# MustaphaMensouri/Distributed-Continuous-Training-with-Airflow-PyTorch-Distributed-DDP-

Measured on AMD Instinct MI355X. Metric: samples/sec (whole node) for weather-MLP DDP, higher is better.
Workload: dtype fp32; 1 GPU; global_batch=4, per_rank_batch=4, parallelism=dp1, optimizer=adam lr=0.01, loss=ce, engine=fused-persistent, dataset_rows=8649, features=5

## Files before the change

distributed-continuous-training-with-airflow-pytorch-distributed-ddp-_amd/csrc/mlp_block5.hip:

```cpp
#include "knobs.h"
#include "mlp_block5_impl.h"
#include "mlp_select.h"

namespace dct {

void mlp_launch_block5_xg(int world, size_t bytes, hipStream_t st, const MlpShape& sh, const MlpArgs& a);
void mlp_launch_block5_b8(size_t bytes, hipStream_t st, const MlpShape& sh, const MlpArgs& a);

static bool b5_xg_world_ok(int w) { return w >= 2 && w <= 8; }

bool mlp_block5_two_micro(const MlpShape& sh, int B) { return B > blk5::B || sh.mlp_block == 8; }

bool mlp_block5_takes(const MlpShape& sh, const MlpLaunchKey& k) {
  const bool aligned = (sh.woff[1] % 4) == 0 && k.p_aligned && k.mv_aligned;
  const bool xg_ok = k.xg_world <= 1 ||
                     (k.mode == 0 && b5_xg_world_ok(k.xg_world) && k.xg_rank >= 0 && k.xg_rank < k.xg_world &&
                      k.xg_bufs && (!k.prof || k.xg_world == 2 || k.xg_world == 4 || k.xg_world == 8));
  const bool b8_ok = !mlp_block5_two_micro(sh, k.B) || !k.prof;
  return aligned && b8_ok && mlp_block5_shape_ok(sh.dims, sh.L, k.B) &&
         ((k.mode == 0 && !k.cursor) || (k.mode == 1 && k.steps == 1 && k.grad_out)) &&
         (k.loss_kind == 0 || k.loss_kind == 1) && !k.pending && (!k.stage || k.mode == 1) && xg_ok;
}

bool mlp_block5_xg_shape_ok(const MlpShape& sh, const MlpLaunchKey& k) {
  return k.mode == 0 && mlp_block5_shape_ok(sh.dims, sh.L, k.B) && mlp_block5_xg_bytes(k.xg_world) > 0;
}

bool mlp_block5_shape_ok(const int* dims, int L, int B) {
  return L == 3 && dims[1] == blk5::H && dims[2] == blk5::H && dims[0] >= 1 && dims[0] <= blk5::DMAX &&
         dims[3] == blk5::C && B >= 1 && B <= blk5::BMAX;
}

size_t mlp_block5_xg_bytes(int world) {
  switch (world) {
    case 2: return (size_t)b5x::Lay<2>::BYTES;
    case 4: return (size_t)b5x::Lay<4>::BYTES;
    case 8: return (size_t)b5x::Lay<8>::BYTES;
    case 3: return (size_t)b5x::Lay<3>::BYTES;
    case 5: return (size_t)b5x::Lay<5>::BYTES;
    case 6: return (size_t)b5x::Lay<6>::BYTES;
    case 7: return (size_t)b5x::Lay<7>::BYTES;
    default: return 0;
  }
}

template <bool WD, int LK, bool PROF = false>
static void b5_launch_sched(int sched, size_t bytes, hipStream_t st, const MlpShape& sh, const MlpArgs& a) {
  using namespace blk5;
  if (sched == 0) return b5_launch<WD, LK, PROF>(bytes, st, sh, a);
#ifdef B5_SCHED_AB
  if constexpr (!WD && LK == 0 && !PROF) {
    constexpr int D = SCHED_DEFAULT;
    constexpr int R = SCHED_R10, E = SCHED_R11;
    constexpr int masks[] = {R, R | SCH_PF_W0, R | SCH_ADAM_SM, R | SCH_DZ2F, R | SCH_DROP_INT, R | SCH_DB2,
                             E & ~SCH_PF_W0,
                             E, E | SCH_LOGIT_RS, E | SCH_INV_BS, E | SCH_ADAM_B02, D & ~SCH_INV_BS};
    bool done = false;
    b5x::static_for<sizeof(masks) / sizeof(masks[0])>([&](auto i) {
      constexpr int M = masks[decltype(i)::value];
      if (!done && sched == B5_SCHED_AB_BASE + M && M != D) {
        b5_launch<WD, LK, false, true, true, 1, -1, 1, M>(bytes, st, sh, a);
        done = true;
      }
    });
    if (done) return;
  }
#endif
  b5_launch<WD, LK, PROF, true, true, 1, -1, 1, SCHED_DEFAULT>(bytes, st, sh, a);
}

hipError_t mlp_launch_block5(const MlpShape& sh, const MlpArgs& a, hipStream_t st) {
  const size_t bytes = (size_t)blk5::LDS_FLOATS * sizeof(float);
  const bool wd = a.wd != 0.f;
  const int sched = knobs().b5_sched;
  if (!mlp_block5_takes(sh, mlp_launch_key(a))) return hipErrorInvalidValue;
  if (mlp_block5_two_micro(sh, a.B)) {
    mlp_launch_block5_b8(bytes, st, sh, a);
  } else if (a.xg_world > 1) {
    mlp_launch_block5_xg(a.xg_world, bytes, st, sh, a);
  } else if (a.mode == 1) {
    if (a.loss_kind == 0) b5_launch<false, 0, false, true, false>(bytes, st, sh, a);
    else b5_launch<false, 1, false, true, false>(bytes, st, sh, a);
  } else if (a.prof) {
    if (a.loss_kind == 0) b5_launch_sched<true, 0, true>(sched, bytes, st, sh, a);
    else b5_launch_sched<true, 1, true>(sched, bytes, st, sh, a);
  } else if (a.loss_kind == 0) {
    if (wd) b5_launch_sched<true, 0>(sched, bytes, st, sh, a);
    else b5_launch_sched<false, 0>(sched, bytes, st, sh, a);
  } else {
    if (wd) b5_launch_sched<true, 1>(sched, bytes, st, sh, a);
    else b5_launch_sched<false, 1>(sched, bytes, st, sh, a);
  }
  return hipGetLastError();
}

}
```

distributed-continuous-training-with-airflow-pytorch-distributed-ddp-_amd/csrc/mlp_block5_impl.h:

```cpp
#pragma once
#include <type_traits>

#include "mlp_block_util.h"

namespace dct {

namespace blk5 {
constexpr int H = 128, NT = 512, NW = 8, KS = 16, DMAX = 8, B = 4, C = 2, MBMAX = 2, BMAX = B * MBMAX;
constexpr int PSTR = 36;
template <int MB>
struct Lds {
  static constexpr int RB = B * MB;
  static constexpr int XT = 0;
  static constexpr int LAB = XT + 3 * DMAX * RB;
  static constexpr int MSK = LAB + (MB == 1 ? 16 : 32);
  static constexpr int LOGP = MSK + 2 * NW * 2;
  static constexpr int H1W = LOGP + 2 * NW * 8;
  static constexpr int H1X = H1W + MB * NW * KS * 4;
  static constexpr int PART = H1X + NW * KS * 4;
  static constexpr int W2L = PART + 2 * H * PSTR;
  static constexpr int B2L = W2L + 2 * H * C;
  static constexpr int ABT = B2L + 8;
  static constexpr int TOTAL = ABT + 4;
  static constexpr int DZF = TOTAL;
  static constexpr int TOTAL_DZF = DZF + 2 * H * 4;
  static_assert((DZF % 4) == 0, "16-B aligned");
  static_assert((H1W % 4) == 0 && (PART % 4) == 0 && (MSK % 4) == 0 && (LAB % 4) == 0 && (W2L % 4) == 0 &&
                    (B2L % 4) == 0 && (H1X % 4) == 0 && (LOGP % 4) == 0,
                "16-B aligned tiles");
};
static_assert(Lds<1>::TOTAL == 11036, "the batch <= 4 layout is round 5's");
constexpr int STG = H * H;
constexpr int LDS_FLOATS = Lds<MBMAX>::TOTAL > 2 * STG ? Lds<MBMAX>::TOTAL : 2 * STG;
static_assert(Lds<1>::TOTAL_DZF <= LDS_FLOATS, "SCH_DZ2F's region inside the launch's LDS");
static_assert(LDS_FLOATS * 4 <= 160 * 1024, "fits the CU");
using Stg = bku::Stage<H, NT>;
constexpr float LOG2E = 1.4426950408889634f, LN2 = 0.6931471805599453f;
constexpr int SCH_DROP = 1, SCH_ADAM_TAB = 2, SCH_WT1 = 8, SCH_WT2 = 16, SCH_WTB = 32;
constexpr int SCH_PRIO_LAT = 64;
constexpr int SCH_PF_W0 = 128, SCH_ADAM_SM = 256, SCH_DZ2F = 512, SCH_DROP_INT = 1024, SCH_DB2 = 2048;
constexpr int SCHED_R10 = SCH_DROP | SCH_ADAM_TAB | SCH_WTB | SCH_PRIO_LAT;
constexpr int SCHED_R11 = SCHED_R10 | SCH_PF_W0 | SCH_ADAM_SM | SCH_DZ2F | SCH_DROP_INT | SCH_DB2;
constexpr int SCH_LOGIT_RS = 4096, SCH_INV_BS = 8192, SCH_ADAM_B02 = 16384;
constexpr int SCHED_DEFAULT = SCHED_R11 | SCH_LOGIT_RS | SCH_INV_BS | SCH_ADAM_B02;
static_assert(SCHED_DEFAULT < 32768, "item masks stay below B5_SCHED_AB_BASE (knobs.h)");
}

namespace b5x {
typedef unsigned int v4u __attribute__((ext_vector_type(4)));
constexpr int SYS = 17;
constexpr int NP = 16, NS = 2;
constexpr int G = blk5::NT * 16;
template <int XW>
struct Lay {
  static constexpr int NO = (NP + XW - 1) / XW;
  static constexpr int RSS = NO + NS;
  static constexpr int AG = 2 * XW * RSS * G;
  static constexpr int LS = AG + 2 * (NP + NS) * G;
  static constexpr int EP = LS + ((2 * XW * 16 + 255) & ~255);
  static constexpr int BYTES = EP + (NP + NS) * 2 * G;
  static __device__ __forceinline__ int rs(int par, int src, int slot) { return ((par * XW + src) * RSS + slot) * G; }
  static __device__ __forceinline__ int ag(int par, int slot) { return AG + (par * (NP + NS) + slot) * G; }
  static __device__ __forceinline__ int ls(int par, int src) { return LS + (par * XW + src) * 16; }
  static __device__ __forceinline__ int ep(int slot, int mv) { return EP + (slot * 2 + mv) * G; }
};
__device__ __forceinline__ void put(__amdgpu_buffer_rsrc_t rs, int off, float x, float y, uint32_t tag) {
  v4u d;
  d.x = __float_as_uint(x);
  d.y = tag;
  d.z = __float_as_uint(y);
  d.w = tag;
  __builtin_amdgcn_raw_buffer_store_b128(d, rs, off, 0, SYS);
}
__device__ __forceinline__ bool get(__amdgpu_buffer_rsrc_t rs, int off, uint32_t tag, float& x, float& y) {
  const v4u d = __builtin_amdgcn_raw_buffer_load_b128(rs, off, 0, SYS);
  x = __uint_as_float(d.x);
  y = __uint_as_float(d.z);
  return (d.y == tag) & (d.w == tag);
}
template <int XW, class T>
__device__ __forceinline__ T pick(const T* v, int rank) {
  T r = v[0];
#pragma unroll
  for (int k = 1; k < XW; ++k) r = rank == k ? v[k] : r;
  return r;
}
template <int V>
using IC = std::integral_constant<int, V>;
template <int N, int I = 0, class F>
__device__ __host__ __forceinline__ void static_for(F&& f) {
  if constexpr (I < N) {
    f(IC<I>{});
    static_for<N, I + 1>(f);
  }
}
}

#define B5STAMP(k)                                              \
  if constexpr (PROF) {                                         \
    const unsigned long long t_ = __builtin_amdgcn_s_memtime(); \
    pacc[(k)] += t_ - t_last;                                   \
    t_last = t_;                                                \
  }

#define B5PRIO(p)                      \
  if constexpr (S_PLAT) {              \
    __builtin_amdgcn_sched_barrier(0); \
    __builtin_amdgcn_s_setprio(p);     \
    __builtin_amdgcn_sched_barrier(0); \
  }

__device__ __forceinline__ uint32_t b5_elem(int li, int r, int u) {
  return ((uint32_t)((li * 64 + r) * 65536 + u) + 0x165667B1u) * 0xC2B2AE3Du;
}
__device__ __forceinline__ float b5_drop(uint32_t seed, uint32_t gstep, uint32_t elem, float p, float scale) {
  uint32_t h = (seed * 0x9E3779B1u) ^ ((gstep + 0x7F4A7C15u) * 0x85EBCA77u);
  h ^= elem;
  h ^= h >> 16;
  h *= 0x7feb352du;
  h ^= h >> 15;
  h *= 0x846ca68bu;
  h ^= h >> 16;
  return u01(h) < p ? 0.f : scale;
}
__device__ __forceinline__ uint32_t b5_drop_thr(float p) { return (uint32_t)ceilf(p * 16777216.0f); }
__device__ __forceinline__ float b5_drop_int(uint32_t seed, uint32_t gstep, uint32_t elem, uint32_t thr, float scale) {
  uint32_t h = (seed * 0x9E3779B1u) ^ ((gstep + 0x7F4A7C15u) * 0x85EBCA77u);
  h ^= elem;
  h ^= h >> 16;
  h *= 0x7feb352du;
  h ^= h >> 15;
  h *= 0x846ca68bu;
  h ^= h >> 16;
  return (h >> 8) < thr ? 0.f : scale;
}

template <bool WD>
__device__ __forceinline__ void adam_pair(float& p0, float g0, float& m0, float& v0, float& p1, float g1, float& m1,
                                          float& v1, float b1, float b2, float wd, float A, float E) {
  if constexpr (WD) { g0 = fmaf(wd, p0, g0); g1 = fmaf(wd, p1, g1); }
  m0 = fmaf(b1, m0, g0);
  m1 = fmaf(b1, m1, g1);
  v0 = fmaf(b2, v0, g0 * g0);
  v1 = fmaf(b2, v1, g1 * g1);
  const float d0 = fmaf(__builtin_amdgcn_sqrtf(v0), A, E), d1 = fmaf(__builtin_amdgcn_sqrtf(v1), A, E);
  const float R = __builtin_amdgcn_rcpf(d0 * d1);
  p0 = fmaf(-m0, d1 * R, p0);
  p1 = fmaf(-m1, d0 * R, p1);
}

__device__ __forceinline__ bku::f32x4_t quad_transpose_mf(const float (&v)[4], const float (&e)[4]) {
  bku::f32x4_t t = (bku::f32x4_t){0.f, 0.f, 0.f, 0.f};
#pragma unroll
  for (int i = 0; i < 4; ++i) t = bku::mfma4(v[i], e[i], t);
  return t;
}

__device__ __forceinline__ float rs_bits2to5(float (&P)[16], int lane) {
  using namespace bku;
#pragma unroll
  for (int i = 0; i < 8; ++i) P[i] = swap32_sum(P[i], P[i + 8]);
#pragma unroll
  for (int i = 0; i < 4; ++i) P[i] = swap16_sum(P[i], P[i + 4]);
  const bool b3 = (lane >> 3) & 1, b2 = (lane >> 2) & 1;
#pragma unroll
  for (int i = 0; i < 2; ++i) {
    const float keep = b3 ? P[i + 2] : P[i], send = b3 ? P[i] : P[i + 2];
    P[i] = keep + dpp<ROR8>(send);
  }
  const float keep = b2 ? P[1] : P[0], send = b2 ? P[0] : P[1];
  const float t4 = dpp<ROR4>(send), t12 = dpp<0x12C>(send);
  return keep + (b2 ? t4 : t12);
}

typedef float v2f __attribute__((ext_vector_type(2)));
template <bool WD>
__device__ __forceinline__ void adam_v2(v2f& p, v2f g, v2f& m, v2f& v, float b1, float b2, float wd, float A, float E) {
  if constexpr (WD) g = (v2f)(wd) * p + g;
  m = (v2f)(b1) * m + g;
  v = (v2f)(b2) * v + g * g;
  const v2f sq = (v2f){__builtin_amdgcn_sqrtf(v.x), __builtin_amdgcn_sqrtf(v.y)};
  const v2f d = sq * (v2f)(A) + (v2f)(E);
  const float R = __builtin_amdgcn_rcpf(d.x * d.y);
  p = p - m * ((v2f){d.y, d.x} * R);
}
template <bool WD>
__device__ __forceinline__ void adam_v2r(v2f& p, v2f g, v2f& m, v2f& v, float b1, float b2, float wd, float A, float E) {
  if constexpr (WD) g = (v2f)(wd) * p + g;
  m = (v2f)(b1) * m + g;
  v = (v2f)(b2) * v + g * g;
  const v2f sq = (v2f){__builtin_amdgcn_sqrtf(v.x), __builtin_amdgcn_sqrtf(v.y)};
  const v2f d = sq * (v2f)(A) + (v2f)(E);
  p = p - m * (v2f){__builtin_amdgcn_rcpf(d.x), __builtin_amdgcn_rcpf(d.y)};
}

template <bool WD, int LK, bool PROF = false, bool DXM = true, bool ADAM = true, int XW = 1, int RK = -1, int MB = 1,
          int SCH = 0>
__global__ __launch_bounds__(blk5::NT, 1) void mlp_block5_kernel(MlpShape sh, MlpArgs a) {
  using namespace blk5;
  using namespace bku;
  static_assert(XW == 1 || (ADAM && XW >= 2 && XW <= 8), "exchange: train mode, 2..8 ranks");
  static_assert(MB >= 1 && MB <= MBMAX, "micro-batches per step");
  static_assert(SCH == 0 || (XW == 1 && MB == 1 && ADAM), "step-schedule items: one-rank train mode, one micro-batch");
  constexpr bool S_DROP = (SCH & SCH_DROP) != 0, S_TAB = (SCH & SCH_ADAM_TAB) != 0;
  constexpr int HQ = DXM ? (SCH / SCH_WT1) & 3 : 0;
  constexpr int HB = DXM ? (SCH / SCH_WTB) & 1 : 0;
  static_assert(HQ + HB <= KS / 4, "W1 has four k-blocks per wave");
  constexpr bool S_PLAT = (SCH & SCH_PRIO_LAT) != 0;
  constexpr bool S_PF = (SCH & SCH_PF_W0) != 0, S_SM = (SCH & SCH_ADAM_SM) != 0, S_DZF = (SCH & SCH_DZ2F) != 0;
  constexpr bool S_DINT = (SCH & SCH_DROP_INT) != 0, S_DB2 = (SCH & SCH_DB2) != 0;
  constexpr bool S_LRS = (SCH & SCH_LOGIT_RS) != 0, S_INVB = (SCH & SCH_INV_BS) != 0, S_B02 = (SCH & SCH_ADAM_B02) != 0;
  constexpr bool S_EV = S_SM || S_B02;
  using LY = Lds<MB>;
  constexpr int RB = LY::RB, XT = LY::XT, LAB = LY::LAB, MSK = LY::MSK, LOGP = LY::LOGP, H1W = LY::H1W;
  constexpr int H1X = LY::H1X, PART = LY::PART, W2L = LY::W2L, B2L = LY::B2L, ABT = LY::ABT, TOTAL = LY::TOTAL;
  constexpr int PS = XW > 1 ? 32 : 16;
  using XL = b5x::Lay<XW>;
  constexpr int NO = XL::NO;
  extern __shared__ __attribute__((aligned(16))) float lds[];
  const int tid = threadIdx.x, w = tid >> 6, l = tid & 63;
  const int D0 = sh.dims[0];
  const int r0 = l & 3;
  const int u = KS * w + (l >> 2);
  const int wo0 = sh.woff[0], bo0 = sh.boff[0], wo1 = sh.woff[1], bo1 = sh.boff[1];
  const int wo2 = sh.woff[2], bo2 = sh.boff[2];
  unsigned long long pacc[PROF ? PS : 1] = {};
  unsigned long long t_last = PROF ? __builtin_amdgcn_s_memtime() : 0ull;
  const unsigned long long t_kstart = t_last;

  const int Bsz = a.B;
  const int fb = tid & (RB - 1), fd = tid / RB;
  const int nel = Bsz * D0;
  int role = 0, pb = 0, pk = 0;
  if (tid < nel) { role = 1; pb = tid / D0; pk = tid - pb * D0; }
  else if (tid < nel + Bsz) { role = 2; pb = tid - nel; }
  const bool stp = !ADAM && a.stage != nullptr;
  uint32_t st_tag = 0u, st_x = 0u, st_lab = 0u;
  if (stp) {
    st_tag = a.stage[0];
    if (tid < RB * DMAX && fd < D0 && fb < Bsz) st_x = a.stage[64 + fb * D0 + fd];
    if (tid < Bsz) st_lab = a.stage[64 + nel + tid];
  }
  const int cur0 = (!ADAM && a.cursor) ? sload(a.cursor) : 0;
  const int bs0 = min(Bsz, a.n_items - cur0 * Bsz);
  const bool first_ok = tid < RB * DMAX && fb < bs0;
  const int rb_raw = a.idx[max(0, min(cur0 * Bsz + (first_ok ? fb : 0), a.n_items - 1))];
  const int rb_first = (first_ok && !stp) ? rb_raw : 0;
  int ridx_next = 0;
  if (!stp && role && (cur0 + 1) * Bsz + pb < a.n_items) ridx_next = a.idx[(cur0 + 1) * Bsz + pb];

  v4f sp[Stg::LD], sm[Stg::LD], sv[Stg::LD];
#pragma unroll
  for (int i = 0; i < Stg::LD; ++i) {
    const int f = wo1 + 4 * (i * NT + tid);
    sp[i] = *reinterpret_cast<const v4f*>(a.p + f);
    if constexpr (ADAM) sm[i] = *reinterpret_cast<const v4f*>(a.m + f);
  }
  if constexpr (ADAM) {
#pragma unroll
    for (int i = 0; i < Stg::LD; ++i) sv[i] = *reinterpret_cast<const v4f*>(a.v + wo1 + 4 * (i * NT + tid));
  }
  float w0[2], m0[2], v0[2];
#pragma unroll
  for (int i = 0; i < 2; ++i) {
    const int d = r0 + 4 * i;
    const bool ok = d < D0;
    const int f = wo0 + u * D0 + (ok ? d : 0);
    w0[i] = ok ? a.p[f] : 0.f;
    m0[i] = (ok && ADAM) ? a.m[f] : 0.f;
    v0[i] = (ok && ADAM) ? a.v[f] : 0.f;
  }
  float pb0 = a.p[bo0 + u], mb0 = ADAM ? a.m[bo0 + u] : 0.f, vb0 = ADAM ? a.v[bo0 + u] : 0.f;
  float pw2[C];
#pragma unroll
  for (int c = 0; c < C; ++c) pw2[c] = a.p[wo2 + c * H + u];
  const bool own_w2 = r0 < C;
  const int fw2 = wo2 + (XW > 1 ? (r0 & 1) : (own_w2 ? r0 : 0)) * H + u;
  float mw2 = ((own_w2 || XW > 1) && ADAM) ? a.m[fw2] : 0.f, vw2 = ((own_w2 || XW > 1) && ADAM) ? a.v[fw2] : 0.f;
  float pb1 = a.p[bo1 + u], mb1 = ADAM ? a.m[bo1 + u] : 0.f, vb1 = ADAM ? a.v[bo1 + u] : 0.f;
  const bool own_b2 = w == 0 && l < C;
  const int fb2 = bo2 + (own_b2 ? l : 0);
  float pb2 = own_b2 ? a.p[fb2] : 0.f, mb2 = (own_b2 && ADAM) ? a.m[fb2] : 0.f, vb2 = (own_b2 && ADAM) ? a.v[fb2] : 0.f;
  const int fbx = r0 == 0 ? bo0 + u : (r0 == 1 ? bo1 + u : bo2 + (l & 1));
  float pbx = 0.f, mbx = 0.f, vbx = 0.f;
  if constexpr (XW > 1) {
    pbx = a.p[fbx];
    mbx = a.m[fbx];
    vbx = a.v[fbx];
  }

  int t0 = a.t0;
  uint32_t step_base = a.step_base;
  if (a.step_counter) {
    t0 = sload(a.step_counter);
    step_base = (uint32_t)t0;
// ... 59 lines not shown
  const float sqc2 = XW > 1 ? a.k_sqc2 : sqrtf(c2);
#pragma unroll
  for (int j = 0; j < 2; ++j)
#pragma unroll
    for (int k = 0; k < KS; ++k) { m1[j][k] *= rc1; v1[j][k] *= rc2; }
#pragma unroll
  for (int i = 0; i < 2; ++i) { m0[i] *= rc1; v0[i] *= rc2; }
  mb0 *= rc1; vb0 *= rc2; mw2 *= rc1; vw2 *= rc2; mb1 *= rc1; vb1 *= rc2; mb2 *= rc1; vb2 *= rc2;
  mbx *= rc1; vbx *= rc2;
  v2f W[2][KS / 2], Mo[2][KS / 2], Vo[2][KS / 2];
#pragma unroll
  for (int j = 0; j < 2; ++j)
#pragma unroll
    for (int h = 0; h < KS / 2; ++h) {
      W[j][h] = (v2f){w1[j][2 * h], w1[j][2 * h + 1]};
      Mo[j][h] = (v2f){m1[j][2 * h], m1[j][2 * h + 1]};
      Vo[j][h] = (v2f){v1[j][2 * h], v1[j][2 * h + 1]};
    }
  const v2f z2 = (v2f){0.f, 0.f};
  v2f PSm = S_SM ? (v2f){0.f, pb1} : z2, MSm = S_SM ? (v2f){mw2, mb1} : z2, VSm = S_SM ? (v2f){vw2, vb1} : z2;
  v2f PW0 = S_SM ? (v2f){w0[0], w0[1]} : z2, MW0 = S_SM ? (v2f){m0[0], m0[1]} : z2, VW0 = S_SM ? (v2f){v0[0], v0[1]} : z2;
  v2f PB02 = S_B02 ? (v2f){pb0, pb2} : z2, MB02 = S_B02 ? (v2f){mb0, mb2} : z2, VB02 = S_B02 ? (v2f){vb0, vb2} : z2;
  const uint32_t inv_bsz = S_INVB ? __builtin_amdgcn_readfirstlane(
                                        __float_as_uint(__builtin_amdgcn_rcpf((float)(Bsz > 0 ? Bsz : 1))))
                                  : 0u;
  const int xrank = XW > 1 ? (RK >= 0 ? RK : a.xg_rank) : 0;
  v2f MoO[NO], VoO[NO];
  __amdgpu_buffer_rsrc_t xrr = __builtin_amdgcn_make_buffer_rsrc((void*)a.xg_recv, 0, 0, 0x00020000), xpr[XW];
  const bool sown = XW == 1 || (__builtin_amdgcn_readfirstlane(w) % XW) == xrank;
  bool xbad = false;
  unsigned long long xticks = 0;
  if constexpr (XW > 1) {
#pragma unroll
    for (int t = 0; t < NO; ++t) {
      v2f cm[XW], cv[XW];
#pragma unroll
      for (int k = 0; k < XW; ++k) {
        const int i = XW * t + k < b5x::NP ? XW * t + k : 0;
        cm[k] = Mo[i >> 3][i & 7];
        cv[k] = Vo[i >> 3][i & 7];
      }
      MoO[t] = b5x::pick<XW>(cm, xrank);
      VoO[t] = b5x::pick<XW>(cv, xrank);
    }
  }
  if constexpr (XW > 1) {
    xrr = __builtin_amdgcn_make_buffer_rsrc((void*)a.xg_recv, 0, XL::BYTES, 0x00020000);
#pragma unroll
    for (int q = 0; q < XW; ++q)
      xpr[q] = __builtin_amdgcn_make_buffer_rsrc((void*)sload_ptr(a.xg_peers, q), 0, XL::BYTES, 0x00020000);
  }
  auto xwait = [&](uint32_t tag, auto&& sweep) -> bool {
    const unsigned long long t_start = __builtin_amdgcn_s_memrealtime();
    for (int spin = 0;; ++spin) {
      asm volatile("" ::: "memory");
      if (__all(sweep())) return true;
      if ((spin & 15) == 15 && (long long)(__builtin_amdgcn_s_memrealtime() - t_start) > a.xg_timeout) {
        if (l == 0) __hip_atomic_store(a.xg_status, tag, __ATOMIC_RELAXED, __HIP_MEMORY_SCOPE_SYSTEM);
        return false;
      }
      __builtin_amdgcn_s_sleep(1);
    }
  };
  const int tb = tid * 16;
  uint32_t el0[MB], el1[MB];
  float f1[MB], f2[MB];
#pragma unroll
  for (int hf = 0; hf < MB; ++hf) {
    el0[hf] = b5_elem(0, r0 + B * hf, u);
    el1[hf] = b5_elem(1, r0 + B * hf, u);
    f1[hf] = b5_drop(a.seed, step_base, el0[hf], p_drop, scale);
    f2[hf] = b5_drop(a.seed, step_base, el1[hf], p_drop, scale);
  }
  const bool pf_wave = !S_PF || __builtin_amdgcn_readfirstlane(w) == 0;
  float* h1x = lds + H1X + w * (KS * 4);
  float eye[4];
#pragma unroll
  for (int i = 0; i < 4; ++i) eye[i] = r0 == i ? 1.f : 0.f;
  const int cb = (l >> 2) & 1;
  int xb = 0;
  float tabA = 0.f, tabE = 0.f;
  if (a.tune == 1 && w >= NW / 2) __builtin_amdgcn_s_setprio(1);
  if (a.tune == 2 && w < NW / 2) __builtin_amdgcn_s_setprio(1);
  if constexpr (PROF) {
    t_last = __builtin_amdgcn_s_memtime();
    pacc[9] = t_last - t_kstart;
  }
  for (int s = 0; s < a.steps; ++s) {
    const int sb = s + cur0;
    const int bs = min(Bsz, a.n_items - sb * Bsz);
    const uint32_t gstep = step_base + (uint32_t)s;
    const int xbn = xb == 2 ? 0 : xb + 1;
    const int pbuf = s & 1, nbuf = pbuf ^ 1;
    const float* xT = lds + XT + xb * DMAX * RB;
    const bool have_next = (s + 1 < a.steps);
    const int bs_next = have_next ? min(Bsz, a.n_items - (sb + 1) * Bsz) : 0;
    uint32_t raw_next = 0u;
    int ridx_next2 = 0;
    if constexpr (S_PF) {
      if (pf_wave) {
        raw_next = pf_base[(size_t)(uint32_t)ridx_next * (uint32_t)pf_stride];
        const int nx2 = min((sb + 2) * Bsz + pb, a.n_items - 1);
        ridx_next2 = a.idx[nx2 < 0 ? 0 : nx2];
      }
    } else {
      raw_next = pf_base[(size_t)ridx_next * pf_stride];
      const int nx2 = min((sb + 2) * Bsz + pb, a.n_items - 1);
      ridx_next2 = a.idx[nx2 < 0 ? 0 : nx2];
    }
    const uint32_t xtag = gstep + 1u;
    const int xpar = (int)(gstep & 1u);
    const int t = t0 + s + 1;
    float dz2m[MB][2][4];
    float dz = 0.f, xbl = 0.f, tls = 0.f;
    float h2 = 0.f, h1 = 0.f;
    float gw0s = 0.f, gw1s = 0.f, gb1s = 0.f, gbs = 0.f, g0s = 0.f, g1s = 0.f, db0s = 0.f;
    float aA = 0.f, aE = 0.f, aEv = 0.f;
    float f1n = 0.f, f2n = 0.f;
    f32x4_t wth[HQ + HB > 0 ? HQ + HB : 1][2];
    v2f GO[NO];
#pragma unroll
    for (int t2 = 0; t2 < NO; ++t2) GO[t2] = (v2f){0.f, 0.f};
    float xg_own = 0.f, xg_bx = 0.f;
    v2f xs_g0 = (v2f){0.f, 0.f}, xs_g1 = (v2f){0.f, 0.f};
    bool abort_step = false;
    auto dw1_pass = [&]() {
#pragma unroll
      for (int q = 0; q < KS / 4; ++q) {
        f32x4_t g[2];
#pragma unroll
        for (int j = 0; j < 2; ++j) g[j] = (f32x4_t){0.f, 0.f, 0.f, 0.f};
#pragma unroll
        for (int hf = 0; hf < MB; ++hf) {
          const float4 hq = *reinterpret_cast<const float4*>(lds + H1W + (hf * NW + w) * (KS * 4) + (4 * q + r0) * 4);
          const float hv[4] = {hq.x, hq.y, hq.z, hq.w};
#pragma unroll
          for (int j = 0; j < 2; ++j)
#pragma unroll
            for (int r = 0; r < 4; ++r) g[j] = mfma4(hv[r], dz2m[hf][j][r], g[j]);
        }

        if constexpr (ADAM && XW > 1) {
#pragma unroll
          for (int j = 0; j < 2; ++j)
#pragma unroll
            for (int h = 0; h < 2; ++h) {
              const int i = 8 * j + 2 * q + h;
              const float gx = g[j][2 * h], gy = g[j][2 * h + 1];
              if ((i % XW) == xrank) GO[i / XW] = (v2f){gx, gy};
              else b5x::put(xpr[i % XW], XL::rs(xpar, (xrank - i % XW + XW) % XW, i / XW) + tb, gx, gy, xtag);
            }
        } else if constexpr (ADAM) {
#pragma unroll
          for (int j = 0; j < 2; ++j)
#pragma unroll
            for (int h = 0; h < 2; ++h)
              adam_v2<WD>(W[j][2 * q + h], (v2f){g[j][2 * h], g[j][2 * h + 1]}, Mo[j][2 * q + h], Vo[j][2 * q + h], a.b1,
                          a.b2, a.wd, aA, aE);
        } else {
#pragma unroll
          for (int j = 0; j < 2; ++j)
            *reinterpret_cast<float4*>(a.grad_out + wo1 + (l + 64 * j) * H + KS * w + 4 * q) =
                make_float4(g[j][0], g[j][1], g[j][2], g[j][3]);
        }
      }
    };

#pragma unroll
    for (int hf = 0; hf < MB; ++hf) {
      const bool last = hf == MB - 1;
      const int mpar = MB == 1 ? pbuf : hf;
      float* h1w = lds + H1W + (hf * NW + w) * (KS * 4);

      const float4 xa = *reinterpret_cast<const float4*>(xT + r0 * RB + B * hf);
      const float4 xc = *reinterpret_cast<const float4*>(xT + (r0 + 4) * RB + B * hf);
      {
        const float wa = S_SM ? PW0.x : w0[0], wc = S_SM ? PW0.y : w0[1];
        const float acc0 = wa * xa.x + wc * xc.x, acc1 = wa * xa.y + wc * xc.y;
        const float acc2 = wa * xa.z + wc * xc.z, acc3 = wa * xa.w + wc * xc.w;
        const bool qb1 = (r0 >> 1) & 1, qb0 = r0 & 1;
        const float k0 = qb1 ? acc2 : acc0, k1 = qb1 ? acc3 : acc1;
        const float s0 = qb1 ? acc0 : acc2, s1 = qb1 ? acc1 : acc3;
        const float e0 = k0 + dpp<QP_X2>(s0), e1 = k1 + dpp<QP_X2>(s1);
        const float kq = qb0 ? e1 : e0, sq = qb0 ? e0 : e1;
        h1 = fmaxf(kq + dpp<QP_X1>(sq) + (S_B02 ? PB02.x : pb0), 0.f) * f1[hf];
        h1w[l] = h1;
        h1x[r0 * KS + (l >> 2)] = h1;
      }
      __builtin_amdgcn_wave_barrier();
      B5STAMP(0)
      {
        f32x4_t cq[2][KS / 4];
#pragma unroll
        for (int q = 0; q < KS / 4; ++q) {
          const float4 hq = *reinterpret_cast<const float4*>(h1x + r0 * KS + 4 * q);
          const float hv[4] = {hq.x, hq.y, hq.z, hq.w};
#pragma unroll
          for (int j = 0; j < 2; ++j) {
            cq[j][q] = (f32x4_t){0.f, 0.f, 0.f, 0.f};
#pragma unroll
            for (int e = 0; e < 4; ++e) cq[j][q] = mfma4(hv[e], W[j][2 * q + (e >> 1)][e & 1], cq[j][q]);
          }
        }
        f32x4_t cj[2];
#pragma unroll
        for (int j = 0; j < 2; ++j) cj[j] = (cq[j][0] + cq[j][1]) + (cq[j][2] + cq[j][3]);
        float* part = lds + PART + mpar * (H * PSTR);
#pragma unroll
        for (int j = 0; j < 2; ++j)
          *reinterpret_cast<float4*>(part + (l + 64 * j) * PSTR + w * 4) = make_float4(cj[j][0], cj[j][1], cj[j][2], cj[j][3]);
      }
      if (hf == 0) {
        if (stp) {
          const int bs_st = min(Bsz, a.n_items - (sb + 1) * Bsz);
          if (role) a.stage[64 + tid] = pb < bs_st ? raw_next : 0u;
          if (tid == 0) a.stage[0] = bs_st > 0 ? (uint32_t)(sb + 2) : 0u;
        }
        if (pf_wave) {
          if (role) {
            const uint32_t v = (have_next && pb < bs_next) ? raw_next : 0u;
            uint32_t* dst = (role == 1) ? reinterpret_cast<uint32_t*>(lds + XT + xbn * DMAX * RB) + pk * RB + pb
                                        : reinterpret_cast<uint32_t*>(lds + LAB) + xbn * RB + pb;
            *dst = v;
          }
          ridx_next = role ? ridx_next2 : 0;
        }
      }
      B5STAMP(1)
      lds_barrier();
      B5STAMP(2)
      B5PRIO(1)
      if constexpr (XW > 1) {
        if (lds[ABT] != 0.f) {
          abort_step = true;
          break;
        }
      }

      const float2 wv0 = *reinterpret_cast<const float2*>(lds + W2L + pbuf * (H * C) + l * C);
      const float2 wv1 = *reinterpret_cast<const float2*>(lds + W2L + pbuf * (H * C) + (l + 64) * C);
      const float b2c = lds[B2L + pbuf * 4 + cb];
      const int lab = reinterpret_cast<const int*>(lds + LAB)[xb * RB + B * hf + r0];
      {
        const float* pr = lds + PART + mpar * (H * PSTR) + u * PSTR + r0;
        float q[NW];
#pragma unroll
        for (int ww = 0; ww < NW; ++ww) q[ww] = pr[4 * ww];
        if constexpr (SCH != 0) {
          __builtin_amdgcn_sched_barrier(0);
          if constexpr (HQ > 0) {
#pragma unroll
            for (int qq = 0; qq < HQ; ++qq)
#pragma unroll
              for (int j = 0; j < 2; ++j) {
                const float wq[4] = {W[j][2 * qq].x, W[j][2 * qq].y, W[j][2 * qq + 1].x, W[j][2 * qq + 1].y};
                wth[qq][j] = quad_transpose_mf(wq, eye);
              }
          }
          if constexpr (S_DROP) {
            uint32_t gnext = gstep + 1u;
            asm volatile("" : "+s"(gnext));
            if constexpr (S_DINT) {
              f1n = b5_drop_int(a.seed, gnext, el0[0], drop_thr, scale);
              f2n = b5_drop_int(a.seed, gnext, el1[0], drop_thr, scale);
            } else {
              f1n = b5_drop(a.seed, gnext, el0[0], p_drop, scale);
              f2n = b5_drop(a.seed, gnext, el1[0], p_drop, scale);
            }
            asm volatile("" : "+v"(f1n), "+v"(f2n));
          }
          if constexpr (S_TAB) {
            const int ti = s & 63;
// ... 231 lines not shown
#pragma unroll
          for (int j = 0; j < 2; ++j) {
            const float wq[4] = {W[j][2 * q].x, W[j][2 * q].y, W[j][2 * q + 1].x, W[j][2 * q + 1].y};
            const f32x4_t wt = q < HQ + HB ? wth[q < HQ + HB ? q : 0][j] : quad_transpose_mf(wq, eye);
            acc[j] = (f32x4_t){0.f, 0.f, 0.f, 0.f};
#pragma unroll
            for (int i = 0; i < 4; ++i) acc[j] = mfma4(wt[i], dzt[j][i], acc[j]);
          }
          const f32x4_t at = acc[0] + acc[1];
#pragma unroll
          for (int m = 0; m < 4; ++m) P[4 * q + m] = at[m];
        }
        dz1 = rs_bits2to5(P, l);
      } else {
#pragma unroll
        for (int p = 0; p < 4; ++p) {
          float P[16];
#pragma unroll
          for (int kk = 0; kk < KS; ++kk)
            P[kk] = W[0][kk >> 1][kk & 1] * dz2m[hf][0][p] + W[1][kk >> 1][kk & 1] * dz2m[hf][1][p];
          const float tot = rs_small<16>(P, l);
          if (r0 == p) dz1 = tot;
        }
      }
      dz1 = h1 > 0.f ? dz1 * scale : 0.f;
      B5PRIO(1)
      {
        const float dq0 = dpp<QB0>(dz1), dq1 = dpp<QB1>(dz1), dq2 = dpp<QB2>(dz1), dq3 = dpp<QB3>(dz1);
        const float g0h = dq0 * xa.x + dq1 * xa.y + dq2 * xa.z + dq3 * xa.w;
        const float g1h = dq0 * xc.x + dq1 * xc.y + dq2 * xc.z + dq3 * xc.w;
        const float dbh = (dq0 + dq1) + (dq2 + dq3);
        g0s = hf == 0 ? g0h : g0s + g0h;
        g1s = hf == 0 ? g1h : g1s + g1h;
        db0s = hf == 0 ? dbh : db0s + dbh;
        if (last) {
          const float g0 = g0s, g1 = g1s;
          if constexpr (ADAM && XW > 1) {
            if (r0 == 0) xg_bx = db0s;
            xs_g0 = (v2f){g0, g1};
            xs_g1 = (v2f){xg_own, xg_bx};
            if (!sown) {
#pragma unroll
              for (int q = 0; q < XW; ++q)
                if (q == __builtin_amdgcn_readfirstlane(w) % XW) {
                  const int rel = (xrank - q + XW) % XW;
                  b5x::put(xpr[q], XL::rs(xpar, rel, NO) + tb, g0, g1, xtag);
                  b5x::put(xpr[q], XL::rs(xpar, rel, NO + 1) + tb, xg_own, xg_bx, xtag);
                }
            }
          } else if constexpr (ADAM) {
            if constexpr (S_SM)
              adam_v2<WD>(PW0, (v2f){g0, g1}, MW0, VW0, a.b1, a.b2, a.wd, aA, aEv);
            else
              adam_pair<WD>(w0[0], g0, m0[0], v0[0], w0[1], g1, m0[1], v0[1], a.b1, a.b2, a.wd, aA, aE);
            if constexpr (S_B02) {
              adam_v2r<WD>(PB02, (v2f){db0s, gbs}, MB02, VB02, a.b1, a.b2, a.wd, aA, aEv);
              if (own_b2) lds[B2L + nbuf * 4 + l] = PB02.y;
            } else {
              adam_scaled<WD>(pb0, db0s, mb0, vb0, a.b1, a.b2, a.wd, aA, S_SM ? aEv : aE);
            }
          } else {
            if (r0 < D0) a.grad_out[wo0 + u * D0 + r0] = g0;
            if (r0 + 4 < D0) a.grad_out[wo0 + u * D0 + r0 + 4] = g1;
            if (r0 == 0) a.grad_out[bo0 + u] = db0s;
          }
        }
      }
    }
    if constexpr (XW > 1) {
      if (abort_step) break;
    }
    B5PRIO(0)
    if constexpr (S_DROP) {
      f1[0] = f1n;
      f2[0] = f2n;
    } else {
#pragma unroll
      for (int hf = 0; hf < MB; ++hf) {
        f1[hf] = b5_drop(a.seed, gstep + 1u, el0[hf], p_drop, scale);
        f2[hf] = b5_drop(a.seed, gstep + 1u, el1[hf], p_drop, scale);
      }
    }
    B5STAMP(7)
    if constexpr (XW == 1) dw1_pass();
    if constexpr (ADAM && XW > 1) {
      const unsigned long long xt0 = __builtin_amdgcn_s_memrealtime();
      const float invw = 1.f / (float)XW;
      do {
        float rv[XW][NO][2], sv[XW][2][2];
        if (!xwait(xtag, [&]() -> bool {
              bool k = true;
#pragma unroll
              for (int q = 1; q < XW; ++q)
#pragma unroll
                for (int t = 0; t < NO; ++t)
                  k &= b5x::get(xrr, XL::rs(xpar, q, t) + tb, xtag, rv[q][t][0], rv[q][t][1]) | (XW * t + xrank >= b5x::NP);
              return k;
            })) {
          xbad = true;
          break;
        }
        B5STAMP(16)
        auto small_sweep = [&]() -> bool {
          bool k = true;
#pragma unroll
          for (int q = 1; q < XW; ++q) {
            k &= b5x::get(xrr, XL::rs(xpar, q, NO) + tb, xtag, sv[q][0][0], sv[q][0][1]);
            k &= b5x::get(xrr, XL::rs(xpar, q, NO + 1) + tb, xtag, sv[q][1][0], sv[q][1][1]);
          }
          return k;
        };
        bool sok = true;
        if (sown) sok = small_sweep();
        v2f WO[NO];
#pragma unroll
        for (int t = 0; t < NO; ++t) {
          v2f cw[XW];
#pragma unroll
          for (int k = 0; k < XW; ++k) {
            const int i = XW * t + k < b5x::NP ? XW * t + k : 0;
            cw[k] = W[i >> 3][i & 7];
          }
          WO[t] = b5x::pick<XW>(cw, xrank);
          v2f gs = GO[t];
#pragma unroll
          for (int q = 1; q < XW; ++q) gs += (v2f){rv[q][t][0], rv[q][t][1]};
          adam_v2<WD>(WO[t], gs * (v2f)(invw), MoO[t], VoO[t], a.b1, a.b2, a.wd, aA, aE);
          const int agoff = XL::ag(xpar, XW * t + xrank) + tb;
          if (XW * t + xrank < b5x::NP) {
#pragma unroll
            for (int q = 0; q < XW; ++q)
              if (q != xrank) b5x::put(xpr[q], agoff, WO[t].x, WO[t].y, xtag);
          }
        }
        B5STAMP(17)
        if (sown && !__all(sok) && !xwait(xtag, small_sweep)) {
          xbad = true;
          break;
        }
        if (sown) {
          v2f s0 = xs_g0, s1 = xs_g1;
#pragma unroll
          for (int q = 1; q < XW; ++q) {
            s0 += (v2f){sv[q][0][0], sv[q][0][1]};
            s1 += (v2f){sv[q][1][0], sv[q][1][1]};
          }
          s0 *= (v2f)(invw);
          s1 *= (v2f)(invw);
          adam_pair<WD>(w0[0], s0.x, m0[0], v0[0], w0[1], s0.y, m0[1], v0[1], a.b1, a.b2, a.wd, aA, aE);
          float pown = (r0 & 1) ? pw2[1] : pw2[0];
          adam_pair<WD>(pown, s1.x, mw2, vw2, pbx, s1.y, mbx, vbx, a.b1, a.b2, a.wd, aA, aE);
          xs_g1.x = pown;
#pragma unroll
          for (int q = 0; q < XW; ++q)
            if (q != xrank) {
              b5x::put(xpr[q], XL::ag(xpar, b5x::NP) + tb, w0[0], w0[1], xtag);
              b5x::put(xpr[q], XL::ag(xpar, b5x::NP + 1) + tb, pown, pbx, xtag);
            }
        }
        B5STAMP(18)
        float av[b5x::NP][2], sa[2][2], lq = 0.f, lq1;
        const int lsrc = l < XW ? l : 0;
        const bool lskip = w != 0 || l >= XW || l == xrank;
        if (!xwait(xtag, [&]() -> bool {
              bool k = true;
#pragma unroll
// ... 113 lines not shown
        vw2 = es[1][1][0]; vbx = es[1][1][1];
      }
    } while (false);
    if (xbad) lds[ABT] = 1.f;
    lds_barrier();
    if (lds[ABT] != 0.f) return;
    mbx *= c1;
    vbx *= c2;
  }
  if (a.step_counter && tid == 0)
    __hip_atomic_store(a.step_counter, t0 + a.steps, __ATOMIC_RELAXED, __HIP_MEMORY_SCOPE_AGENT);
  if constexpr (!ADAM) {
    if (a.cursor && tid == 0) __hip_atomic_store(a.cursor, cur0 + a.steps, __ATOMIC_RELAXED, __HIP_MEMORY_SCOPE_AGENT);
    return;
  }

  int lo = l, uo = u, to = tid;
  asm volatile("" : "+v"(lo), "+v"(uo), "+v"(to));
#pragma unroll
  for (int j = 0; j < 2; ++j)
#pragma unroll
    for (int h = 0; h < KS / 2; ++h) {
      w1[j][2 * h] = W[j][h].x; w1[j][2 * h + 1] = W[j][h].y;
      m1[j][2 * h] = Mo[j][h].x; m1[j][2 * h + 1] = Mo[j][h].y;
      v1[j][2 * h] = Vo[j][h].x; v1[j][2 * h + 1] = Vo[j][h].y;
    }
#pragma unroll
  for (int j = 0; j < 2; ++j)
#pragma unroll
    for (int k = 0; k < KS; ++k) { m1[j][k] *= c1; v1[j][k] *= c2; }
#pragma unroll
  for (int i = 0; i < 2; ++i) { m0[i] *= c1; v0[i] *= c2; }
  mb0 *= c1; vb0 *= c2; mw2 *= c1; vw2 *= c2; mb1 *= c1; vb1 *= c2; mb2 *= c1; vb2 *= c2;
  lds_barrier();
  Stg::own<KS>(lds, w1, lo, KS / 4 * w);
  Stg::own<KS>(lds + STG, m1, lo, KS / 4 * w);
  lds_barrier();
  Stg::store(a.p + wo1, lds, to);
  Stg::store(a.m + wo1, lds + STG, to);
  lds_barrier();
  Stg::own<KS>(lds, v1, lo, KS / 4 * w);
  lds_barrier();
  Stg::store(a.v + wo1, lds, to);
  const int r0o = lo & 3;
#pragma unroll
  for (int i = 0; i < 2; ++i) {
    const int d = r0o + 4 * i;
    if (d < D0) {
      const int f = wo0 + uo * D0 + d;
      a.p[f] = w0[i];
      a.m[f] = m0[i];
      a.v[f] = v0[i];
    }
  }
  if constexpr (XW > 1) {
    if (r0o < 2 || (w == 0 && (lo == 2 || lo == 3))) {
      a.p[fbx] = pbx; a.m[fbx] = mbx; a.v[fbx] = vbx;
    }
    if (own_w2) {
      const int f = wo2 + r0o * H + uo;
      a.p[f] = (r0o & 1) ? pw2[1] : pw2[0]; a.m[f] = mw2; a.v[f] = vw2;
    }
  } else {
    if (r0o == 0) {
      a.p[bo0 + uo] = pb0; a.m[bo0 + uo] = mb0; a.v[bo0 + uo] = vb0;
      a.p[bo1 + uo] = pb1; a.m[bo1 + uo] = mb1; a.v[bo1 + uo] = vb1;
    }
    if (own_w2) {
      const int f = wo2 + r0o * H + uo;
      a.p[f] = (r0o & 1) ? pw2[1] : pw2[0]; a.m[f] = mw2; a.v[f] = vw2;
    }
    if (own_b2) { a.p[fb2] = pb2; a.m[fb2] = mb2; a.v[fb2] = vb2; }
  }
  if constexpr (PROF) {
    asm volatile("s_waitcnt vmcnt(0)" ::: "memory");
    pacc[10] = __builtin_amdgcn_s_memtime() - t_last;
    if (l == 0) {
#pragma unroll
      for (int i = 0; i < PS - 1; ++i) atomicAdd(a.prof + w * PS + i, pacc[i]);
    }
  }
}
#undef B5STAMP
#undef B5PRIO

template <bool WD, int LK, bool PROF = false, bool DXM = true, bool ADAM = true, int XW = 1, int RK = -1, int MB = 1,
          int SCH = 0>
inline void b5_launch(size_t bytes, hipStream_t st, const MlpShape& sh, const MlpArgs& a) {
  static const hipError_t attr = hipFuncSetAttribute((const void*)mlp_block5_kernel<WD, LK, PROF, DXM, ADAM, XW, RK, MB, SCH>,
                                                     hipFuncAttributeMaxDynamicSharedMemorySize, (int)bytes);
  (void)attr;
  hipLaunchKernelGGL((mlp_block5_kernel<WD, LK, PROF, DXM, ADAM, XW, RK, MB, SCH>), dim3(1), dim3(blk5::NT), bytes, st, sh, a);
}


}
```

Measured before the change: 1.259 million samples/s.

## Compute next step's first-layer activations ahead, double-buffering the h1 tile

Adds a schedule bit that computes the next step's layer-1 forward (x load, W0 dot, bias, ReLU, dropout) right after the dropout-mask refresh, before the dw1 pass, into a second LDS h1 tile selected by step parity. The next iteration reuses these carried registers instead of recomputing at the head of the step, which is meant to hide that latency behind the backward and Adam work. It is enabled in the default schedule. It adds a second LDS tile, extra live registers, and a dependency on the W0 values in use before the optimizer update, so any staleness would change the maths.

```diff
diff --git a/distributed-continuous-training-with-airflow-pytorch-distributed-ddp-_amd/csrc/mlp_block5.hip b/distributed-continuous-training-with-airflow-pytorch-distributed-ddp-_amd/csrc/mlp_block5.hip
--- a/distributed-continuous-training-with-airflow-pytorch-distributed-ddp-_amd/csrc/mlp_block5.hip
+++ b/distributed-continuous-training-with-airflow-pytorch-distributed-ddp-_amd/csrc/mlp_block5.hip
@@ -51,10 +51,10 @@
 #ifdef B5_SCHED_AB
   if constexpr (!WD && LK == 0 && !PROF) {
     constexpr int D = SCHED_DEFAULT;
-    constexpr int R = SCHED_R10, E = SCHED_R11;
+    constexpr int R = SCHED_R10, E = SCHED_R11, T = SCHED_R12;
     constexpr int masks[] = {R, R | SCH_PF_W0, R | SCH_ADAM_SM, R | SCH_DZ2F, R | SCH_DROP_INT, R | SCH_DB2,
                              E & ~SCH_PF_W0,
-                             E, E | SCH_LOGIT_RS, E | SCH_INV_BS, E | SCH_ADAM_B02, D & ~SCH_INV_BS};
+                             E, E | SCH_LOGIT_RS, E | SCH_INV_BS, E | SCH_ADAM_B02, T & ~SCH_INV_BS, T};
     bool done = false;
     b5x::static_for<sizeof(masks) / sizeof(masks[0])>([&](auto i) {
       constexpr int M = masks[decltype(i)::value];
diff --git a/distributed-continuous-training-with-airflow-pytorch-distributed-ddp-_amd/csrc/mlp_block5_impl.h b/distributed-continuous-training-with-airflow-pytorch-distributed-ddp-_amd/csrc/mlp_block5_impl.h
--- a/distributed-continuous-training-with-airflow-pytorch-distributed-ddp-_amd/csrc/mlp_block5_impl.h
+++ b/distributed-continuous-training-with-airflow-pytorch-distributed-ddp-_amd/csrc/mlp_block5_impl.h
@@ -24,7 +24,9 @@
   static constexpr int TOTAL = ABT + 4;
   static constexpr int DZF = TOTAL;
   static constexpr int TOTAL_DZF = DZF + 2 * H * 4;
-  static_assert((DZF % 4) == 0, "16-B aligned");
+  static constexpr int H1W2 = TOTAL_DZF;
+  static constexpr int TOTAL_F1A = H1W2 + NW * KS * 4;
+  static_assert((DZF % 4) == 0 && (H1W2 % 4) == 0, "16-B aligned");
   static_assert((H1W % 4) == 0 && (PART % 4) == 0 && (MSK % 4) == 0 && (LAB % 4) == 0 && (W2L % 4) == 0 &&
                     (B2L % 4) == 0 && (H1X % 4) == 0 && (LOGP % 4) == 0,
                 "16-B aligned tiles");
@@ -33,6 +35,7 @@
 constexpr int STG = H * H;
 constexpr int LDS_FLOATS = Lds<MBMAX>::TOTAL > 2 * STG ? Lds<MBMAX>::TOTAL : 2 * STG;
 static_assert(Lds<1>::TOTAL_DZF <= LDS_FLOATS, "SCH_DZ2F's region inside the launch's LDS");
+static_assert(Lds<1>::TOTAL_F1A <= LDS_FLOATS, "SCH_F1_AHEAD's second h1 tile inside the launch's LDS");
 static_assert(LDS_FLOATS * 4 <= 160 * 1024, "fits the CU");
 using Stg = bku::Stage<H, NT>;
 constexpr float LOG2E = 1.4426950408889634f, LN2 = 0.6931471805599453f;
@@ -42,7 +45,9 @@
 constexpr int SCHED_R10 = SCH_DROP | SCH_ADAM_TAB | SCH_WTB | SCH_PRIO_LAT;
 constexpr int SCHED_R11 = SCHED_R10 | SCH_PF_W0 | SCH_ADAM_SM | SCH_DZ2F | SCH_DROP_INT | SCH_DB2;
 constexpr int SCH_LOGIT_RS = 4096, SCH_INV_BS = 8192, SCH_ADAM_B02 = 16384;
-constexpr int SCHED_DEFAULT = SCHED_R11 | SCH_LOGIT_RS | SCH_INV_BS | SCH_ADAM_B02;
+constexpr int SCHED_R12 = SCHED_R11 | SCH_LOGIT_RS | SCH_INV_BS | SCH_ADAM_B02;
+constexpr int SCH_F1_AHEAD = 4;
+constexpr int SCHED_DEFAULT = SCHED_R12 | SCH_F1_AHEAD;
 static_assert(SCHED_DEFAULT < 32768, "item masks stay below B5_SCHED_AB_BASE (knobs.h)");
 }
 
@@ -110,6 +115,23 @@
     __builtin_amdgcn_sched_barrier(0); \
   }
 
+#define B5_F1(XA, XC, H1V, XR, XO, FK, H1WP)                                                \
+  XA = *reinterpret_cast<const float4*>(XR + r0 * RB + XO);                                 \
+  XC = *reinterpret_cast<const float4*>(XR + (r0 + 4) * RB + XO);                           \
+  {                                                                                         \
+    const float wa = S_SM ? PW0.x : w0[0], wc = S_SM ? PW0.y : w0[1];                       \
+    const float acc0 = wa * XA.x + wc * XC.x, acc1 = wa * XA.y + wc * XC.y;                 \
+    const float acc2 = wa * XA.z + wc * XC.z, acc3 = wa * XA.w + wc * XC.w;                 \
+    const bool qb1 = (r0 >> 1) & 1, qb0 = r0 & 1;                                           \
+    const float k0 = qb1 ? acc2 : acc0, k1 = qb1 ? acc3 : acc1;                             \
+    const float s0 = qb1 ? acc0 : acc2, s1 = qb1 ? acc1 : acc3;                             \
+    const float e0 = k0 + dpp<QP_X2>(s0), e1 = k1 + dpp<QP_X2>(s1);                         \
+    const float kq = qb0 ? e1 : e0, sq = qb0 ? e0 : e1;                                     \
+    H1V = fmaxf(kq + dpp<QP_X1>(sq) + (S_B02 ? PB02.x : pb0), 0.f) * (FK);                  \
+    (H1WP)[l] = H1V;                                          \
+    h1x[r0 * KS + (l >> 2)] = H1V;                                            \
+  }
+
 __device__ __forceinline__ uint32_t b5_elem(int li, int r, int u) {
   return ((uint32_t)((li * 64 + r) * 65536 + u) + 0x165667B1u) * 0xC2B2AE3Du;
 }
@@ -211,6 +233,7 @@
   constexpr bool S_DINT = (SCH & SCH_DROP_INT) != 0, S_DB2 = (SCH & SCH_DB2) != 0;
   constexpr bool S_LRS = (SCH & SCH_LOGIT_RS) != 0, S_INVB = (SCH & SCH_INV_BS) != 0, S_B02 = (SCH & SCH_ADAM_B02) != 0;
   constexpr bool S_EV = S_SM || S_B02;
+  constexpr bool S_F1A = (SCH & SCH_F1_AHEAD) != 0;
   using LY = Lds<MB>;
   constexpr int RB = LY::RB, XT = LY::XT, LAB = LY::LAB, MSK = LY::MSK, LOGP = LY::LOGP, H1W = LY::H1W;
   constexpr int H1X = LY::H1X, PART = LY::PART, W2L = LY::W2L, B2L = LY::B2L, ABT = LY::ABT, TOTAL = LY::TOTAL;
@@ -436,6 +459,13 @@
   float tabA = 0.f, tabE = 0.f;
   if (a.tune == 1 && w >= NW / 2) __builtin_amdgcn_s_setprio(1);
   if (a.tune == 2 && w < NW / 2) __builtin_amdgcn_s_setprio(1);
+  auto h1w_par = [&](int par) { return lds + H1W + par * (LY::H1W2 - H1W) + w * (KS * 4); };
+  float4 xa_c = make_float4(0.f, 0.f, 0.f, 0.f), xc_c = xa_c;
+  float h1_c = 0.f;
+  if constexpr (S_F1A) {
+    B5_F1(xa_c, xc_c, h1_c, (lds + XT), 0, f1[0], h1w_par(0))
+    __builtin_amdgcn_wave_barrier();
+  }
   if constexpr (PROF) {
     t_last = __builtin_amdgcn_s_memtime();
     pacc[9] = t_last - t_kstart;
@@ -486,7 +516,8 @@
         for (int j = 0; j < 2; ++j) g[j] = (f32x4_t){0.f, 0.f, 0.f, 0.f};
 #pragma unroll
         for (int hf = 0; hf < MB; ++hf) {
-          const float4 hq = *reinterpret_cast<const float4*>(lds + H1W + (hf * NW + w) * (KS * 4) + (4 * q + r0) * 4);
+          const float* h1t = S_F1A ? h1w_par(pbuf) : lds + H1W + (hf * NW + w) * (KS * 4);
+          const float4 hq = *reinterpret_cast<const float4*>(h1t + (4 * q + r0) * 4);
           const float hv[4] = {hq.x, hq.y, hq.z, hq.w};
 #pragma unroll
           for (int j = 0; j < 2; ++j)
@@ -526,22 +557,15 @@
       const int mpar = MB == 1 ? pbuf : hf;
       float* h1w = lds + H1W + (hf * NW + w) * (KS * 4);
 
-      const float4 xa = *reinterpret_cast<const float4*>(xT + r0 * RB + B * hf);
-      const float4 xc = *reinterpret_cast<const float4*>(xT + (r0 + 4) * RB + B * hf);
-      {
-        const float wa = S_SM ? PW0.x : w0[0], wc = S_SM ? PW0.y : w0[1];
-        const float acc0 = wa * xa.x + wc * xc.x, acc1 = wa * xa.y + wc * xc.y;
-        const float acc2 = wa * xa.z + wc * xc.z, acc3 = wa * xa.w + wc * xc.w;
-        const bool qb1 = (r0 >> 1) & 1, qb0 = r0 & 1;
-        const float k0 = qb1 ? acc2 : acc0, k1 = qb1 ? acc3 : acc1;
-        const float s0 = qb1 ? acc0 : acc2, s1 = qb1 ? acc1 : acc3;
-        const float e0 = k0 + dpp<QP_X2>(s0), e1 = k1 + dpp<QP_X2>(s1);
-        const float kq = qb0 ? e1 : e0, sq = qb0 ? e0 : e1;
-        h1 = fmaxf(kq + dpp<QP_X1>(sq) + (S_B02 ? PB02.x : pb0), 0.f) * f1[hf];
-        h1w[l] = h1;
-        h1x[r0 * KS + (l >> 2)] = h1;
-      }
-      __builtin_amdgcn_wave_barrier();
+      float4 xa, xc;
+      if constexpr (S_F1A) {
+        xa = xa_c;
+        xc = xc_c;
+        h1 = h1_c;
+      } else {
+        B5_F1(xa, xc, h1, xT, B * hf, f1[hf], h1w)
+        __builtin_amdgcn_wave_barrier();
+      }
       B5STAMP(0)
       {
         f32x4_t cq[2][KS / 4];
@@ -939,6 +963,7 @@
       }
     }
     B5STAMP(7)
+    if constexpr (S_F1A) { B5_F1(xa_c, xc_c, h1_c, (lds + XT + xbn * DMAX * RB), 0, f1[0], h1w_par(nbuf)) }
     if constexpr (XW == 1) dw1_pass();
     if constexpr (ADAM && XW > 1) {
       const unsigned long long xt0 = __builtin_amdgcn_s_memrealtime();
@@ -1218,6 +1243,7 @@
   }
 }
 #undef B5STAMP
+#undef B5_F1
 #undef B5PRIO
 
 template <bool WD, int LK, bool PROF = false, bool DXM = true, bool ADAM = true, int XW = 1, int RK = -1, int MB = 1,
```

After: 1.266 million samples/s (median of 6 runs). No clear change (+0.6%).
